# BogdanDIA/gr-dvbt

Measured on AMD Instinct MI355X. Metric: RX Msamples/s (baseband in -> TS out), higher is better.
Workload: dtype u8 (Viterbi/RS) + f32 (front end)

## Files before the change

gr_dvbt_amd/csrc/k_viterbi3.hpp:

```cpp
#pragma once
#include <hip/hip_runtime.h>
#include <stdint.h>
#include <limits.h>
#include <string.h>
#include "dvbt_tables.hpp"
#include "k_backend.hpp"

namespace dvbt {

inline VitParams make_vit_params(const Dims &d, int bsize, int chunk_bytes)
{
  VitParams v; memset(&v, 0, sizeof v);
  v.m = d.m; v.k = d.k; v.n = d.n; v.plen = d.plen; v.ntb = d.ntb; v.bsize = bsize;
  v.d_nsymbols = bsize * d.n / d.m; v.d_nbits = 2 * d.k * bsize;
  v.chunk_bytes = chunk_bytes > 0 ? chunk_bytes : 768; v.payload = d.payload; v.warm = 72;
  memcpy(v.punct, d.punct, 16); memcpy(v.prefix, d.prefix, 16);
  v.punct_mask = 0; v.prefix_nib = 0;
  for (int i = 0; i < d.plen; i++) { v.punct_mask |= (unsigned)d.punct[i] << i; v.prefix_nib |= (unsigned long long)d.prefix[i] << (4 * i); }
  v.magic_plen = ~0ull / (unsigned)d.plen + 1; v.magic_m = ~0ull / (unsigned)d.m + 1;
  for (int i = 0; i < 64; i++) v.punct_rep |= (unsigned long long)d.punct[i % d.plen] << i;
  v.magic16_plen = (65536u + (unsigned)d.plen - 1) / (unsigned)d.plen;
  return v;
}

#define DPP_XOR1 0xB1
#define DPP_XOR2 0x4E
#define DPP_HALF_MIRROR 0x141
#define DPP_ROR8 0x128
#define DPP_MIRROR 0x140

__device__ __forceinline__ int rotl6(int c, int p) { return ((c << p) | (c >> (6 - p))) & 63; }

#ifndef V3_WGW_N
#define V3_WGW_N 4
#endif
constexpr int V3_WGW = V3_WGW_N;
#ifndef V3_EXP
#define V3_EXP 0
#endif
constexpr int V3_WARM = 72;
constexpr int V3_WARM_MAX = 1152;
static_assert(V3_WARM == 72, "make_vit_params (above) presets VitParams.warm to the default");
constexpr int V3_BLK = 24;
constexpr int V3_RINGW = 64;
constexpr int V3_WAVES_PER_CU = 4 * 2;
constexpr int V3_CBW = 17;

typedef short v3pk __attribute__((ext_vector_type(2)));
__device__ __forceinline__ v3pk pk(int x) { return __builtin_bit_cast(v3pk, x); }
__device__ __forceinline__ int ipk(v3pk x) { return __builtin_bit_cast(int, x); }
__device__ __forceinline__ int pk_add(int a, int b) { return ipk(pk(a) + pk(b)); }
__device__ __forceinline__ int pk_sub(int a, int b) { return ipk(pk(a) - pk(b)); }
__device__ __forceinline__ int pk_max(int a, int b) { return ipk(__builtin_elementwise_max(pk(a), pk(b))); }
__device__ __forceinline__ int pk_min(int a, int b) { return ipk(__builtin_elementwise_min(pk(a), pk(b))); }
template <int CTRL> __device__ __forceinline__ int dppb(int v) { return __builtin_amdgcn_update_dpp(0, v, CTRL, 0xf, 0xf, true); }
__device__ __forceinline__ int vconst(int c) { int x; asm("v_mov_b32 %0, %1" : "=v"(x) : "s"(c)); return x; }
__device__ __forceinline__ int pk_max_swap(int a, int b) { int r; asm("v_pk_max_i16 %0, %1, %2 op_sel:[0,1] op_sel_hi:[1,0]" : "=v"(r) : "v"(a), "v"(b)); return r; }

struct V3Lane {
  unsigned sel[6][2];
  int bias8[6][2];
  int kc[3][2];
  int org[2];
  int arm_mid[3][2];
  int arm_b2[3][2];
  int arm_org[3][2];
};

__device__ __forceinline__ int v3_phys(int a) { const int a2 = (a >> 2) & 1; return (a & 8) | (a2 << 2) | ((a & 3) ^ (a2 ? 3 : 0)); }
__device__ __forceinline__ int v3_log(int p) { const int q = p & 7, a2 = (q >> 2) & 1; return (p & 8) | (a2 << 2) | ((q ^ (a2 ? 7 : 0)) & 3); }
__device__ __forceinline__ int v3_cell_of_z(int z) { return ((z & 2) << 4) | ((z & 1) << 4) | v3_log(z >> 2); }
__device__ __forceinline__ int v3_z_of_cell(int c) { return v3_phys(c & 15) * 4 + ((c >> 5) & 1) * 2 + ((c >> 4) & 1); }

__device__ __forceinline__ int v3_upper(int P, int r, int h, int a) { const int c = (r << 5) | (h << 4) | a; return (c >> (5 - P)) & 1; }
__device__ inline void v3_init_lane(int pl, V3Lane &L)
{
  const int a = v3_log(pl);
  for (int r = 0; r < 2; r++) {
    for (int P = 0; P < 6; P++) {
      unsigned idx[2];
      for (int h = 0; h < 2; h++) {
        const int c = (r << 5) | (h << 4) | a, i = rotl6(c, P) & 31;
        const int c0 = ((i >> 2) ^ (i >> 1) ^ i) & 1;
        const int c1 = ((i >> 4) ^ (i >> 2) ^ (i >> 1)) & 1;
        idx[h] = (unsigned)(c0 | (c1 << 1));
      }
      L.sel[P][r] = 0x0c | (idx[0] << 8) | (0x0cu << 16) | (idx[1] << 24);
      L.bias8[P][r] = (v3_upper(P, r, 0, a) << 8) | (v3_upper(P, r, 1, a) << 24);
    }
    L.org[r] = (pl * 4 + 2 * r) | ((pl * 4 + 2 * r + 1) << 16);
    for (int e = 0; e < 3; e++) {
      const int P0 = 2 * e;
      const int s0 = rotl6((r << 5) | a, P0), s1 = rotl6((r << 5) | 16 | a, P0);
      L.kc[e][r] = ((63 - s0) | ((63 - s1) << 16)) | (L.bias8[P0][r] ^ 0x01000100);
      const int b2 = ((s0 >> 4) << 6) | (((s1 >> 4) << 6) << 16);
      L.arm_mid[e][r] = (L.bias8[(P0 + 3) % 6][r] >> 2) | (L.bias8[(P0 + 4) % 6][r] >> 1) | L.bias8[(P0 + 5) % 6][r];
      L.arm_org[e][r] = L.org[r] | (L.bias8[P0][r] >> 2) | (L.bias8[P0 + 1][r] >> 1) | L.bias8[(P0 + 2) % 6][r];
      L.arm_b2[e][r] = b2 | L.bias8[P0][r];
    }
  }
  for (int r = 0; r < 2; r++) {
    for (int P = 0; P < 6; P++) asm("" : "+v"(L.bias8[P][r]));
    for (int e = 0; e < 3; e++) { asm("" : "+v"(L.kc[e][r])); asm("" : "+v"(L.arm_mid[e][r])); asm("" : "+v"(L.arm_b2[e][r])); asm("" : "+v"(L.arm_org[e][r])); }
  }
}

template <int P, int ST> __device__ __forceinline__ void v3_step(int (&v)[2], unsigned W, const V3Lane &L, int (&raw)[2])
{
  int X[2], Y[2], mx[2];
  const int D0 = (int)__builtin_amdgcn_perm(0u, W, L.sel[P][0]);
  X[0] = pk_add(v[0], D0); Y[0] = pk_sub(v[0], D0);
  if (P == 0 || P == 4) { X[1] = pk_add(v[1], D0); Y[1] = pk_sub(v[1], D0); }
  else if (P == 2 || P == 3) { X[1] = pk_sub(v[1], D0); Y[1] = pk_add(v[1], D0); }
  else {
    const int D1 = (int)__builtin_amdgcn_perm(0u, W, L.sel[P][1]);
    X[1] = pk_add(v[1], D1); Y[1] = pk_sub(v[1], D1);
  }
  if (P == 0) { mx[0] = pk_max(X[0], Y[1]); mx[1] = pk_max(X[1], Y[0]); }
  else if (P == 1) { mx[0] = pk_max_swap(X[0], Y[0]); mx[1] = pk_max_swap(X[1], Y[1]); }
  else {
#pragma unroll
    for (int r = 0; r < 2; r++)
      mx[r] = pk_max(X[r], P == 2 ? dppb<DPP_ROR8>(Y[r]) : P == 3 ? dppb<DPP_HALF_MIRROR>(Y[r]) : P == 4 ? dppb<DPP_XOR2>(Y[r]) : dppb<DPP_XOR1>(Y[r]));
  }
  constexpr int PN = (P + 1) % 6;
#pragma unroll
  for (int r = 0; r < 2; r++) {
    if (ST == 0) v[r] = mx[r];
    else if (ST == 3) v[r] = (mx[r] & (int)0xfe3ffe3f) | L.arm_mid[((PN + 3) % 6) / 2][r];
    else if (ST == 1) v[r] = (mx[r] & (int)0xfe3ffe3f) | L.arm_b2[PN / 2][r];
    else if (ST == 4) v[r] = (mx[r] & (int)0xfefffeff) | L.bias8[PN][r];
    else { raw[r] = mx[r]; v[r] = (mx[r] & (int)0xfe00fe00) | L.arm_org[PN / 2][r]; }
  }
}

#if V3_EXP & 64
#define V3_YIELD() asm volatile("s_nop 3" ::: "memory")
#else
#define V3_YIELD()
#endif

__device__ __forceinline__ int lo16(int x) { return (x << 16) >> 16; }
__device__ __forceinline__ int hi16(int x) { return x >> 16; }
template <int CTRL> __device__ __forceinline__ int max_dpp(int v) { return max(v, dppb<CTRL>(v)); }
template <int CTRL> __device__ __forceinline__ int min_dpp(int v) { return min(v, dppb<CTRL>(v)); }

template <int PE, bool RENORM> __device__ __forceinline__ int v3_window_end(int (&v)[2], const V3Lane &L)
{
  const int kp = pk_max((v[0] & (int)0xfe00fe00) | L.kc[PE / 2][0], (v[1] & (int)0xfe00fe00) | L.kc[PE / 2][1]);
  int k = max(lo16(kp), hi16(kp));
  k = max_dpp<DPP_XOR1>(k); k = max_dpp<DPP_XOR2>(k); k = max_dpp<DPP_HALF_MIRROR>(k); k = max_dpp<DPP_MIRROR>(k);
  if (RENORM) {
    const unsigned sub = (unsigned)((k & ~0x1ff) - (48 << 8));
    const int mn = (int)__builtin_amdgcn_perm(sub, sub, 0x01000100u);
    v[0] = pk_sub(v[0], mn); v[1] = pk_sub(v[1], mn);
  }
  return k;
}

template <int NW> constexpr int V3_ROW = NW * 4 * 64;
template <int NW> constexpr int V3_RMASK = (V3_RINGW * V3_ROW<NW> - 1) & ~63;
struct V3Trace {
  int z[2];
  int wsh[2];
  int oph[2];
  bool ok[2];
  int oend[2];
  int ob[2];
};
__device__ __forceinline__ void v3_hop_read(const V3Trace &T, const unsigned char *tab, unsigned (&t)[2])
{
#pragma unroll
  for (int q = 0; q < 2; q++) t[q] = tab[T.z[q]];
}
template <int NW> __device__ __forceinline__ void v3_hop_merge(V3Trace &T, const unsigned (&t)[2])
{
#pragma unroll
  for (int q = 0; q < 2; q++) {
    T.wsh[q] -= V3_ROW<NW>;
    asm("v_bfi_b32 %0, %1, %2, %3" : "=v"(T.z[q]) : "s"(V3_RMASK<NW>), "v"(T.wsh[q]), "v"(t[q]));
  }
}
template <int NW> __device__ __forceinline__ void v3_hop(V3Trace &T, const unsigned char *tab) { unsigned t[2]; v3_hop_read(T, tab, t); v3_hop_merge<NW>(T, t); }
__device__ __forceinline__ void v3_trace_out(const V3Trace &T, const unsigned char *tab, uint8_t *outb)
{
#pragma unroll
  for (int q = 0; q < 2; q++) {
    const unsigned t = tab[T.z[q]];
    const int sstart = rotl6(v3_cell_of_z((int)(t & 63u)), T.oph[q]);
    if (T.ok[q]) outb[T.ob[q]] = (unsigned char)((sstart << 2) | (t >> 6));
  }
}

__device__ __forceinline__ void v3_load_words(const unsigned *wp_, unsigned (&W)[8])
{
  const uint4 *wp = reinterpret_cast<const uint4 *>(wp_);
  const uint4 t0 = wp[0], t1 = wp[1];
  W[0] = t0.x; W[1] = t0.y; W[2] = t0.z; W[3] = t0.w; W[4] = t1.x; W[5] = t1.y; W[6] = t1.z; W[7] = t1.w;
}
template <int V6, bool HOPS, int HOP0, int NTB, int NW, bool PREF> __device__ __forceinline__ void v3_fwd_window(int (&v)[2], const V3Lane &L, const unsigned *wrow, unsigned char *tab, unsigned char *tabw,
                                                                                           unsigned char *bests, int j0, int dd, int pl, V3Trace &T, unsigned (&W)[8], unsigned (&Wn)[8])
{
  constexpr bool HOPA = HOPS && HOP0 + 2 * V6 < NTB - 1, HOPB = HOPS && HOP0 + 2 * V6 + 1 < NTB - 1;
  unsigned th[2];
  if (HOPA) v3_hop_read(T, tab, th);
  const int jr = (j0 + V6) & (V3_RINGW - 1);
#if V3_EXP & 256
  for (int i = 0; i < 8; i++) { W[i] = (unsigned)(j0 * 0x01010101 + i * 0x00020406 + pl); asm volatile("" : "+v"(W[i])); }
#else
  if (PREF) v3_load_words(wrow + (V6 + 1) * 8, Wn);
#endif
  constexpr int P0 = (8 * V6) % 6;
  int raw[2];
#if V3_EXP & 32
  if (V6 & 1) __builtin_amdgcn_s_setprio(1); else __builtin_amdgcn_s_setprio(0);
#endif
#if V3_EXP & 128
  __builtin_amdgcn_s_sleep(1);
#endif
  v3_step<(P0 + 0) % 6, 0>(v, W[0], L, raw); V3_YIELD(); v3_step<(P0 + 1) % 6, 0>(v, W[1], L, raw); V3_YIELD(); v3_step<(P0 + 2) % 6, 3>(v, W[2], L, raw); V3_YIELD();
  if (HOPA) { v3_hop_merge<NW>(T, th); if (HOPB) v3_hop_read(T, tab, th); }
  v3_step<(P0 + 3) % 6, 0>(v, W[3], L, raw); V3_YIELD(); v3_step<(P0 + 4) % 6, 0>(v, W[4], L, raw); V3_YIELD(); v3_step<(P0 + 5) % 6, 1>(v, W[5], L, raw); V3_YIELD();
  v3_step<(P0 + 6) % 6, 4>(v, W[6], L, raw); V3_YIELD(); v3_step<(P0 + 7) % 6, 2>(v, W[7], L, raw);
  if (HOPB) v3_hop_merge<NW>(T, th);
  if (!(V3_EXP & 4)) *reinterpret_cast<unsigned *>(tabw + jr * V3_ROW<NW>) = __builtin_amdgcn_perm((unsigned)raw[1], (unsigned)raw[0], 0x06040200u);
  if (V3_EXP & 2) { if (raw[0] == 0x12345) bests[jr] = 1; return; }
  const int s = v3_window_end<(P0 + 2) % 6, (V6 & 1) == 1>(v, L);
  bests[dd * V3_RINGW + jr] = (unsigned char)s;
}
template <bool HOPS, int HOP0, int NTB, int NW, bool MORE> __device__ __forceinline__ void v3_fwd_six(int (&v)[2], const V3Lane &L, const unsigned *wrow, unsigned char *tab, unsigned char *tabw,
                                                                                  unsigned char *bests, int j0, int dd, int pl, V3Trace &T, unsigned (&Wa)[8], unsigned (&Wb)[8])
{
  v3_fwd_window<0, HOPS, HOP0, NTB, NW, true>(v, L, wrow, tab, tabw, bests, j0, dd, pl, T, Wa, Wb); v3_fwd_window<1, HOPS, HOP0, NTB, NW, true>(v, L, wrow, tab, tabw, bests, j0, dd, pl, T, Wb, Wa);
  v3_fwd_window<2, HOPS, HOP0, NTB, NW, true>(v, L, wrow, tab, tabw, bests, j0, dd, pl, T, Wa, Wb); v3_fwd_window<3, HOPS, HOP0, NTB, NW, true>(v, L, wrow, tab, tabw, bests, j0, dd, pl, T, Wb, Wa);
  v3_fwd_window<4, HOPS, HOP0, NTB, NW, true>(v, L, wrow, tab, tabw, bests, j0, dd, pl, T, Wa, Wb); v3_fwd_window<5, HOPS, HOP0, NTB, NW, MORE>(v, L, wrow, tab, tabw, bests, j0, dd, pl, T, Wb, Wa);
}

#if V3_EXP & 16
__device__ unsigned long long *v3_dbg;
#endif

constexpr int V3_SLOT = 32;
constexpr int V3_CTL_CHUNKS = 0;
constexpr int V3_CTL_MISMATCH = 1;
constexpr int V3_CTL_CONFLICT = 2;
constexpr int V3_CTL_UNPROVEN = 3;
constexpr int V3_CTL_SEQ = 4;
constexpr int V3_CTL_ACC = 8;
constexpr int V3_CTL_HDR = 16;
struct V3Aux {
  int *snap;
  int *ctl;
  long long cap;
  long long grid0;
  const int *carry_in;
  int *carry_out; int carry_rel;
  int debug;
};
__device__ __forceinline__ int *v3_own(const V3Aux &ax, long long c) { return ax.snap + (3 * c) * V3_SLOT; }
__device__ __forceinline__ int *v3_pred(const V3Aux &ax, long long c) { return ax.snap + (3 * c + 1) * V3_SLOT; }
__device__ __forceinline__ int *v3_fix(const V3Aux &ax, long long c) { return ax.snap + (3 * c + 2) * V3_SLOT; }
inline size_t v3_snap_words(long long cap) { return (size_t)(cap + 2) * 3 * V3_SLOT; }
inline size_t v3_ctl_words(long long cap) { return (size_t)V3_CTL_HDR + 2 * (size_t)(cap + 2); }

struct V3Lds { unsigned char *tab; unsigned *wbuf; unsigned char *bests; const unsigned *lut; int wv; };
__device__ __forceinline__ void v3_init_lut(unsigned *lut, int lane)
{
  if (lane < 16) {
    const int k0 = (lane >> 2) & 1, k1 = (lane >> 3) & 1, t1 = (lane >> 1) & 1, t0 = lane & 1;
    const int u0 = k0 ? 1 - 2 * t1 : 0, u1 = k1 ? 1 - 2 * (k0 ? t0 : t1) : 0;
    const unsigned d0 = (unsigned)(2 * (u0 + u1)) & 0xff, d1 = (unsigned)(2 * (-u0 + u1)) & 0xff;
    const unsigned d2 = (unsigned)(2 * (u0 - u1)) & 0xff, d3 = (unsigned)(2 * (-u0 - u1)) & 0xff;
    lut[lane] = d0 | (d1 << 8) | (d2 << 16) | (d3 << 24);
  }
}

template <int NTB, int WARM, int MODE, int NW>
__device__ __forceinline__ void v3_decode(const uint8_t *__restrict__ in, uint8_t *__restrict__ out, long long total_steps, long long total_out, const VitParams &vp,
                                          long long in_base, long long out_lo, long long b0, bool dec_active, const V3Lds &S, const V3Lane &L, int (&v)[2], int (&endv)[2],
                                          int *own, int *predn, const int *inject, int *carry, int carry_rel)
{
  unsigned char *const tab = S.tab; unsigned *const wbuf = S.wbuf; unsigned char *const bests = S.bests; const unsigned *const lut = S.lut;
  unsigned *const cbits = wbuf;
  constexpr int V3_CBS = V3_BLK * 8;
  static_assert(V3_CBW <= V3_CBS, "bit stream does not fit the step-word row");
  const int lane = threadIdx.x & 63, dd = lane >> 4, pl = lane & 15;
  const int rowl = S.wv * 256 + dd * 64;
  unsigned char *const tabw = tab + rowl + pl * 4;
  const int B = vp.chunk_bytes, m = vp.m;
  constexpr int ntb = NTB;
  const long long b1 = (b0 + B < total_out) ? b0 + B : total_out;
  const int warm = MODE == 2 ? 0 : WARM > 0 ? WARM : vp.warm;
  const long long w0 = b0 + 2 - warm;
  const int J = ((warm + B + ntb - 1 + V3_BLK - 1) / V3_BLK) * V3_BLK;
  const long long n_in_bytes = (total_steps * 2 / vp.plen * vp.n + vp.m - 1) / vp.m;
  const int nload = ((384 + 2 * m - 2) / m + 3 + 15) / 16;

  uint8_t *const outb = out + (b0 - out_lo);
  const int ob_end = !dec_active ? INT_MIN : (int)(b1 - b0 > INT_MIN / 2 ? b1 - b0 : INT_MIN / 2);
  const int ob_lo = MODE != 1 || out_lo <= b0 ? 0 : (int)(out_lo - b0 < INT_MAX / 2 ? out_lo - b0 : INT_MAX / 2);
  const long long tb0 = 8 * (w0 - 1) - 2;
  constexpr int BLKBITS = 2 * 8 * V3_BLK;
  const int inc_q = BLKBITS / vp.plen, inc_ph = BLKBITS - inc_q * vp.plen;
  const unsigned magic16_m = (65536u + (unsigned)m - 1) / (unsigned)m;

  int u_first, u_last;
  {
    const long long r = total_steps - 8 * V3_BLK - tb0;
    int first = tb0 >= 0 ? 0 : (int)((-tb0 + 7) >> 3 < J ? (-tb0 + 7) >> 3 : J), last = !dec_active || r < 0 ? -1 : (int)(r >> 3 < J ? r >> 3 : J);
    u_first = max(max(__builtin_amdgcn_readlane(first, 0), __builtin_amdgcn_readlane(first, 16)), max(__builtin_amdgcn_readlane(first, 32), __builtin_amdgcn_readlane(first, 48)));
    u_last = min(min(__builtin_amdgcn_readlane(last, 0), __builtin_amdgcn_readlane(last, 16)), min(__builtin_amdgcn_readlane(last, 32), __builtin_amdgcn_readlane(last, 48)));
  }
  int ph0 = 0, bo0 = 0, off = 0; long long byte0 = 0; uint4 q = make_uint4(0, 0, 0, 0);
  auto stage_load = [&](int jb) {
    const long long tb = tb0 + (long long)jb * 8;
    if (jb > 0 && jb - V3_BLK >= u_first) {
      const int pf0 = (int)((vp.prefix_nib >> (4 * ph0)) & 15ull);
      ph0 += inc_ph;
      const int wrap = ph0 >= vp.plen ? 1 : 0;
      ph0 -= wrap ? vp.plen : 0;
      const int r = bo0 + (inc_q + wrap) * vp.n + (int)((vp.prefix_nib >> (4 * ph0)) & 15ull) - pf0;
      const int dby = (int)(((unsigned)r * magic16_m) >> 16);
      bo0 = r - dby * m; byte0 += dby;
    } else {
      const unsigned long long pbit = 2ull * (unsigned long long)(tb > 0 ? tb : 0);
      const unsigned long long pq = __umul64hi(pbit, vp.magic_plen);
      ph0 = (int)(pbit - pq * (unsigned)vp.plen);
      const unsigned long long rb = pq * (unsigned)vp.n + ((vp.prefix_nib >> (4 * ph0)) & 15ull);
      const unsigned long long by = __umul64hi(rb, vp.magic_m);
      byte0 = (long long)by; bo0 = (int)(rb - by * (unsigned)m);
    }
    off = (int)(((unsigned long long)(uintptr_t)in + (unsigned long long)(byte0 - in_base)) & 3ull);
    const long long src = byte0 - off + pl * 16;
    q = make_uint4(0, 0, 0, 0);
    if (dec_active && pl < nload) {
      if (src >= in_base && src + 16 <= n_in_bytes) q = *reinterpret_cast<const uint4 *>(in + (src - in_base));
      else {
        unsigned w[4] = {0, 0, 0, 0};
        for (int i = 0; i < 16; i++) {
          const long long bb = src + i;
          const unsigned bv = (bb >= in_base && bb < n_in_bytes) ? in[bb - in_base] : 0;
          w[i >> 2] |= bv << (8 * (i & 3));
        }
        q = make_uint4(w[0], w[1], w[2], w[3]);
      }
    }
  };
  auto stage_words = [&](int jb) {
    {
      const unsigned mk = (1u << m) - 1;
      auto grp = [&](unsigned d) { return ((d & mk) << (3 * m)) | (((d >> 8) & mk) << (2 * m)) | (((d >> 16) & mk) << m) | ((d >> 24) & mk); };
      const unsigned g0 = grp(q.x), g1 = grp(q.y), g2 = grp(q.z), g3 = grp(q.w);
      unsigned *cb = cbits + dd * V3_CBS;
      if (pl < nload) {
        if (m == 2) cb[pl] = (g0 << 24) | (g1 << 16) | (g2 << 8) | g3;
        else if (m == 4) { cb[2 * pl] = (g0 << 16) | g1; cb[2 * pl + 1] = (g2 << 16) | g3; }
        else { cb[3 * pl] = (g0 << 8) | (g1 >> 16); cb[3 * pl + 1] = (g1 << 16) | (g2 >> 8); cb[3 * pl + 2] = (g2 << 24) | g3; }
      }
    }
    __builtin_amdgcn_fence(__ATOMIC_SEQ_CST, "wavefront");
    constexpr int SPL = V3_BLK * 8 / 16;
    const long long tb = tb0 + (long long)jb * 8;
    const int ub0 = pl * SPL;
    int lo = 0, hi = SPL;
    int x = ph0 + 2 * ub0;
    if (jb < u_first || jb > u_last) {
      const long long tbr = tb > 0 ? tb : 0;
      const long long t = tb + ub0;
      if (t < 0) lo = (-t < SPL) ? (int)(-t) : SPL;
      const long long rem = total_steps - t;
      hi = !dec_active ? 0 : rem <= 0 ? 0 : rem < SPL ? (int)rem : SPL;
      if (hi < lo) hi = lo;
      x = ph0 + 2 * (int)((t + lo) - tbr);
      if (x < 0) x = 0;
    }
    const int dq = (int)(((unsigned)x * vp.magic16_plen) >> 16);
    const int ph = x - dq * vp.plen;
    const int pos = off * m + bo0 + dq * vp.n + (int)((vp.prefix_nib >> (4 * ph)) & 15ull) - (int)((vp.prefix_nib >> (4 * ph0)) & 15ull);
    const unsigned kmask = ((unsigned)(vp.punct_rep >> ph) << (2 * lo)) & (((1u << (2 * hi)) - 1u) & ~((1u << (2 * lo)) - 1u));
    const unsigned *cb = cbits + dd * V3_CBS;
    const unsigned cw0 = cb[pos >> 5], cw1 = cb[(pos >> 5) + 1];
    unsigned win = (unsigned)(((((unsigned long long)cw0) << 32) | cw1) >> (32 - (pos & 31)));
#pragma unroll
    for (int i = 0; i < SPL; i++) {
      const unsigned k2 = (kmask >> (2 * i)) & 3u;
      const unsigned idx = (k2 << 2) | (win >> 30);
      win <<= __popc(k2);
      wbuf[dd * (V3_BLK * 8) + ub0 + i] = lut[idx];
    }
    __builtin_amdgcn_fence(__ATOMIC_SEQ_CST, "wavefront");
  };
  V3Trace T;
  int tph[2];
#pragma unroll
  for (int c = 0; c < 2; c++) { T.oend[c] = c * 16 + pl < V3_BLK ? ob_end : INT_MIN; tph[c] = 2 * ((c * 16 + pl + 1) % 3); T.oph[c] = 2 * ((c * 16 + pl + 3 * ntb - (ntb - 1)) % 3); }
  static_assert(V3_BLK % 3 == 0, "phases per lane");
  auto trace_init = [&](int jp) {
#pragma unroll
    for (int c = 0; c < 2; c++) {
      const int jj = jp + c * 16 + pl;
      T.ob[c] = jj - (warm + ntb - 1);
      T.ok[c] = T.ob[c] >= ob_lo && T.ob[c] < T.oend[c];
      const int sb = 63 - (bests[dd * V3_RINGW + (jj & (V3_RINGW - 1))] & 63);
      T.wsh[c] = jj * V3_ROW<NW> + rowl;
      T.z[c] = v3_z_of_cell(((sb | (sb << 6)) >> tph[c]) & 63) | (T.wsh[c] & V3_RMASK<NW>);
    }
  };

  stage_load(0);
  for (int jb = 0; jb < J; jb += V3_BLK) {
    if (MODE == 1 && dec_active) {
      if (jb == warm) { if (inject) { v[0] = inject[0]; v[1] = inject[1]; } own[0] = v[0]; own[1] = v[1]; }
      if (jb == warm + B) { predn[0] = v[0]; predn[1] = v[1]; }
      if (carry && jb == warm + carry_rel) { carry[0] = v[0]; carry[1] = v[1]; }
    }
    if (MODE == 2) {
      if (jb == 0 && dec_active) { own[0] = v[0]; own[1] = v[1]; }
      if (jb == B) { endv[0] = v[0]; endv[1] = v[1]; }
      if (carry && dec_active && jb == carry_rel) { carry[0] = v[0]; carry[1] = v[1]; }
    }
    if (!(V3_EXP & 8) || jb == 0) stage_words(jb);
    if (jb + V3_BLK < J && !(V3_EXP & 8)) stage_load(jb + V3_BLK);
    const bool tr = jb > 0 && !(V3_EXP & 1);
    if (tr) trace_init(jb - V3_BLK);
    const unsigned *wrow = wbuf + dd * (V3_BLK * 8);
    unsigned Wa[8], Wb[8];
    v3_load_words(wrow, Wa);
    if (tr) {
      v3_fwd_six<true, 0, NTB, NW, true>(v, L, wrow, tab, tabw, bests, jb, dd, pl, T, Wa, Wb);
      v3_fwd_six<true, 12, NTB, NW, true>(v, L, wrow + 48, tab, tabw, bests, jb + 6, dd, pl, T, Wa, Wb);
      v3_trace_out(T, tab, outb);
    } else {
      v3_fwd_six<false, 0, NTB, NW, true>(v, L, wrow, tab, tabw, bests, jb, dd, pl, T, Wa, Wb);
      v3_fwd_six<false, 0, NTB, NW, true>(v, L, wrow + 48, tab, tabw, bests, jb + 6, dd, pl, T, Wa, Wb);
    }
    static_assert(V3_BLK == 24, "the second half of the block is written out: two groups of six windows, straight-line like the first half");
    v3_fwd_six<false, 0, NTB, NW, true>(v, L, wrow + 96, tab, tabw, bests, jb + 12, dd, pl, T, Wa, Wb);
    v3_fwd_six<false, 0, NTB, NW, false>(v, L, wrow + 144, tab, tabw, bests, jb + 18, dd, pl, T, Wa, Wb);
  }
  __builtin_amdgcn_fence(__ATOMIC_SEQ_CST, "wavefront");
  trace_init(J - V3_BLK);
  for (int h = 0; h < ntb - 1; h++) v3_hop<NW>(T, tab);
  v3_trace_out(T, tab, outb);
}

template <int NW> struct V3Shared {
  alignas(16) unsigned char tab[V3_RINGW * V3_ROW<NW>];
  alignas(16) unsigned wbuf[NW][4 * V3_BLK * 8];
  unsigned char bests[NW][4 * V3_RINGW];
  unsigned lut[16];
};
static_assert(sizeof(V3Shared<4>) <= 81920 && V3_RMASK<4> == 0xffc0 && V3_RMASK<1> == 0x3fc0, "two four-wave workgroups per CU beside the symbol kernel's 76 KB");
#define V3_LDS_DECL(NW) __shared__ V3Shared<NW> sh_;
#define V3_LDS(NW, wv) V3Lds{sh_.tab, sh_.wbuf[wv], sh_.bests[wv], sh_.lut, wv}

template <int NTB, int WARM = V3_WARM, int MODE = 0> __global__ __launch_bounds__(64 * V3_WGW) void viterbi3_kernel(const uint8_t *__restrict__ in, uint8_t *__restrict__ out, const RxState *st,
                                                      long long steps_fixed, VitParams vp, V3Aux ax, long long in_base, long long out_lo)
{
  V3_LDS_DECL(V3_WGW)
  const int wv = V3_WGW > 1 ? (int)(threadIdx.x >> 6) : 0;
  const V3Lds S = V3_LDS(V3_WGW, wv);
  const int lane = threadIdx.x & 63, dd = lane >> 4, pl = lane & 15;
  const long long total_steps = st ? st->n_vit_steps : steps_fixed;
  const long long total_out = total_steps / 8 - vp.ntb;
  const int B = vp.chunk_bytes;
  if (MODE == 1 && blockIdx.x == 0 && threadIdx.x == 0) {
    ax.ctl[V3_CTL_MISMATCH] = 0; ax.ctl[V3_CTL_CONFLICT] = 0; ax.ctl[V3_CTL_UNPROVEN] = -1; ax.ctl[V3_CTL_SEQ] = 0;
  }
  const long long grid0 = MODE == 1 ? ax.grid0 : out_lo;
  const long long chunk0 = ((long long)blockIdx.x * V3_WGW + wv) * 4;
  if (grid0 + chunk0 * B >= total_out) return;
  const long long c = chunk0 + dd, b0 = grid0 + c * B;
  const bool dec_active = b0 < total_out;
  v3_init_lut(sh_.lut, lane);
#if V3_EXP & 16
  const unsigned long long dbg_t0 = wall_clock64();
#endif
  V3Lane L; v3_init_lane(pl, L);
  int v[2] = {L.arm_org[0][0], L.arm_org[0][1]}, endv[2];
  int *own = nullptr, *predn = nullptr, *carry = nullptr; const int *inject = nullptr;
  if (MODE == 1) {
    own = v3_own(ax, c) + 2 * pl; predn = v3_pred(ax, c + 1) + 2 * pl;
    if (c == 0 && ax.carry_in) inject = ax.carry_in + 2 * pl;
    if (ax.carry_out && b0 + B >= total_out) carry = ax.carry_out + 2 * pl;
  }
  v3_decode<NTB, WARM, MODE, V3_WGW>(in, out, total_steps, total_out, vp, in_base, out_lo, b0, dec_active, S, L, v, endv, own, predn, inject, carry, ax.carry_rel);
#if V3_EXP & 16
  if (lane == 0) {
    unsigned id, xcc;
    asm volatile("s_getreg_b32 %0, hwreg(HW_REG_HW_ID)" : "=s"(id));
    asm volatile("s_getreg_b32 %0, hwreg(HW_REG_XCC_ID)" : "=s"(xcc));
    unsigned long long *d = v3_dbg + 3 * ((long long)blockIdx.x * V3_WGW + wv);
    d[0] = (id & 0xffffu) | ((xcc & 0xfu) << 16); d[1] = dbg_t0; d[2] = wall_clock64();
  }
#endif
}

__device__ __forceinline__ long long v3_nchunks(long long total_out, long long grid0, int B) { return total_out > grid0 ? (total_out - grid0 + B - 1) / B : 0; }
__device__ __forceinline__ bool v3_slots_equal(const int *a_, const int *b_)
{
  const int4 *a = reinterpret_cast<const int4 *>(a_), *b = reinterpret_cast<const int4 *>(b_);
  bool same = true;
#pragma unroll
  for (int i = 0; i < 8; i++) { const int4 x = a[i], y = b[i]; same = same && x.x == y.x && x.y == y.y && x.z == y.z && x.w == y.w; }
  return same;
}

__global__ __launch_bounds__(256) void viterbi_check_kernel(V3Aux ax, const RxState *st, long long steps_fixed, VitParams vp, int pass)
{
  const long long total_steps = st ? st->n_vit_steps : steps_fixed;
  const long long nch = v3_nchunks(total_steps / 8 - vp.ntb, ax.grid0, vp.chunk_bytes);
  if (blockIdx.x == 0 && threadIdx.x == 0) { ax.ctl[V3_CTL_CHUNKS] = (int)(nch < INT_MAX ? nch : INT_MAX); if (pass == 1) ax.ctl[V3_CTL_UNPROVEN] = 0; }
  const long long c = (long long)blockIdx.x * 256 + threadIdx.x + 1;
  if (c >= nch || c > ax.cap) return;
  const bool same = v3_slots_equal(v3_own(ax, c), v3_pred(ax, c));
  if (pass == 0) {
    ax.ctl[V3_CTL_HDR + (ax.cap + 2) + c] = 0;
    if (!same) ax.ctl[V3_CTL_HDR + atomicAdd(ax.ctl + V3_CTL_MISMATCH, 1)] = (int)c;
  }
}
__global__ __launch_bounds__(256) void viterbi_count_kernel(V3Aux ax, const RxState *st, long long steps_fixed, VitParams vp)
{
  const long long total_steps = st ? st->n_vit_steps : steps_fixed;
  const long long nch = v3_nchunks(total_steps / 8 - vp.ntb, ax.grid0, vp.chunk_bytes);
  const long long c = (long long)blockIdx.x * 256 + threadIdx.x + 1;
  if (c >= nch || c > ax.cap) return;
  if (!v3_slots_equal(v3_own(ax, c), v3_pred(ax, c))) atomicAdd(ax.ctl + V3_CTL_UNPROVEN, 1);
}

__device__ __forceinline__ bool v3_row_equal(const int (&a)[2], const int (&b)[2], int dd)
{
  const unsigned long long ne = __ballot(a[0] != b[0] || a[1] != b[1]);
  return ((ne >> (16 * dd)) & 0xffffull) == 0;
}

template <int NTB, int NW> __device__ __forceinline__ void v3_repair_rows(const uint8_t *__restrict__ in, uint8_t *__restrict__ out, long long total_steps, const VitParams &vp, const V3Aux &ax,
                                                                  long long in_base, long long out_lo, const V3Lds &S, const V3Lane &L, long long rows, long long row0, int n)
{
  const int lane = threadIdx.x & 63, dd = lane >> 4, pl = lane & 15;
  const long long total_out = total_steps / 8 - vp.ntb;
  const int B = vp.chunk_bytes;
  const long long nch = v3_nchunks(total_out, ax.grid0, B);
  for (long long i0 = row0; i0 < n; i0 += rows) {
    const bool act = i0 + dd < n;
    const long long c = act ? ax.ctl[V3_CTL_HDR + i0 + dd] : 1;
    const long long b0 = ax.grid0 + c * B;
    int v[2], endv[2] = {0, 0};
    { const int *p = v3_pred(ax, c) + 2 * pl; v[0] = p[0]; v[1] = p[1]; }
    int *carry = (act && ax.carry_out && b0 + B >= total_out) ? ax.carry_out + 2 * pl : nullptr;
    v3_decode<NTB, 0, 2, NW>(in, out, total_steps, total_out, vp, in_base, out_lo, b0, act && b0 < total_out, S, L, v, endv, v3_own(ax, c) + 2 * pl, nullptr, nullptr, carry, ax.carry_rel);
    int pn[2] = {endv[0], endv[1]};
    if (act && c + 1 < nch) { const int *p = v3_pred(ax, c + 1) + 2 * pl; pn[0] = p[0]; pn[1] = p[1]; }
    if (!v3_row_equal(endv, pn, dd) || ((ax.debug & 1) && act && c + 1 < nch)) {
      int *f = v3_fix(ax, c + 1) + 2 * pl; f[0] = endv[0]; f[1] = endv[1];
      if (pl == 0) { ax.ctl[V3_CTL_HDR + (ax.cap + 2) + c + 1] = 1; atomicAdd(ax.ctl + V3_CTL_CONFLICT, 1); }
    }
    __builtin_amdgcn_fence(__ATOMIC_SEQ_CST, "wavefront");
  }
}
template <int NTB> __global__ __launch_bounds__(64 * V3_WGW) void viterbi_repair_kernel(const uint8_t *__restrict__ in, uint8_t *__restrict__ out, const RxState *st,
                                                      long long steps_fixed, VitParams vp, V3Aux ax, long long in_base, long long out_lo)
{
  V3_LDS_DECL(V3_WGW)
  const int n = ax.ctl[V3_CTL_MISMATCH];
  const int wv = V3_WGW > 1 ? (int)(threadIdx.x >> 6) : 0;
  const long long rows = (long long)gridDim.x * V3_WGW * 4, row0 = ((long long)blockIdx.x * V3_WGW + wv) * 4;
  if (row0 >= n) return;
  const V3Lds S = V3_LDS(V3_WGW, wv);
  v3_init_lut(sh_.lut, threadIdx.x & 63);
  V3Lane L; v3_init_lane(threadIdx.x & 15, L);
  v3_repair_rows<NTB, V3_WGW>(in, out, st ? st->n_vit_steps : steps_fixed, vp, ax, in_base, out_lo, S, L, rows, row0, n);
}

template <int NTB, int NW> __device__ __forceinline__ void v3_seq_walk(const uint8_t *__restrict__ in, uint8_t *__restrict__ out, long long total_steps, const VitParams &vp, const V3Aux &ax,
                                                               long long in_base, long long out_lo, const V3Lds &S, const V3Lane &L, int force)
{
  const int lane = threadIdx.x & 63, dd = lane >> 4, pl = lane & 15;
  if (lane == 0) { ax.ctl[V3_CTL_ACC] += ax.ctl[V3_CTL_CHUNKS]; ax.ctl[V3_CTL_ACC + 1] += ax.ctl[V3_CTL_MISMATCH]; }
  if (!force && ax.ctl[V3_CTL_CONFLICT] == 0) return;
  const long long total_out = total_steps / 8 - vp.ntb;
  const int B = vp.chunk_bytes;
  long long nch = v3_nchunks(total_out, ax.grid0, B);
  if (nch > ax.cap) nch = ax.cap;
  const int *cflag = ax.ctl + V3_CTL_HDR + (ax.cap + 2);
  int done = 0;
  long long pos = 0;
  for (;;) {
    long long cn = -1;
    for (long long c0 = pos + 1; c0 < nch && cn < 0; c0 += 64) {
      const long long c = c0 + lane;
      bool hit = false;
      if (c < nch) hit = cflag[c] != 0 || (force && !v3_slots_equal(v3_own(ax, c), v3_pred(ax, c)));
      const unsigned long long b = __ballot(hit);
      if (b) cn = c0 + __builtin_ctzll(b);
    }
    if (cn < 0) break;
    long long c = cn;
    int v[2];
    { const int *p = (cflag[c] ? v3_fix(ax, c) : v3_pred(ax, c)) + 2 * pl; v[0] = p[0]; v[1] = p[1]; }
    for (;;) {
      const long long b0 = ax.grid0 + c * B;
      const bool act = dd == 0;
      int st0[2] = {v[0], v[1]}, endv[2] = {0, 0};
      if (act) { int *p = v3_pred(ax, c) + 2 * pl; p[0] = v[0]; p[1] = v[1]; }
      int *carry = (act && ax.carry_out && b0 + B >= total_out) ? ax.carry_out + 2 * pl : nullptr;
      v3_decode<NTB, 0, 2, NW>(in, out, total_steps, total_out, vp, in_base, out_lo, b0, act, S, L, st0, endv, v3_own(ax, c) + 2 * pl, nullptr, nullptr, carry, ax.carry_rel);
      __builtin_amdgcn_fence(__ATOMIC_SEQ_CST, "wavefront");
      done++;
      if (c + 1 >= nch) { pos = nch; break; }
      int on[2]; { const int *p = v3_own(ax, c + 1) + 2 * pl; on[0] = p[0]; on[1] = p[1]; }
      const bool eq = (__ballot(on[0] != endv[0] || on[1] != endv[1]) & 0xffffull) == 0;
      if (act) { int *p = v3_pred(ax, c + 1) + 2 * pl; p[0] = endv[0]; p[1] = endv[1]; }
      if (eq) { pos = c + 1; break; }
      c++; v[0] = endv[0]; v[1] = endv[1];
    }
  }
  if (lane == 0) { ax.ctl[V3_CTL_SEQ] = done; ax.ctl[V3_CTL_ACC + 2] += done; }
}
template <int NTB> __global__ __launch_bounds__(64) void viterbi_repair_seq_kernel(const uint8_t *__restrict__ in, uint8_t *__restrict__ out, const RxState *st,
                                                      long long steps_fixed, VitParams vp, V3Aux ax, long long in_base, long long out_lo, int force)
{
  V3_LDS_DECL(1)
  const V3Lds S = V3_LDS(1, 0);
  v3_init_lut(sh_.lut, threadIdx.x & 63);
  V3Lane L; v3_init_lane(threadIdx.x & 15, L);
  v3_seq_walk<NTB, 1>(in, out, st ? st->n_vit_steps : steps_fixed, vp, ax, in_base, out_lo, S, L, force);
}

constexpr long long V3_FIX_SMALL = 1024;
template <int NTB> __global__ __launch_bounds__(64 * V3_WGW) void viterbi_fix_kernel(const uint8_t *__restrict__ in, uint8_t *__restrict__ out, const RxState *st,
                                                      long long steps_fixed, VitParams vp, V3Aux ax, long long in_base, long long out_lo, int force)
{
  V3_LDS_DECL(V3_WGW)
  const int wv = V3_WGW > 1 ? (int)(threadIdx.x >> 6) : 0;
  const long long total_steps = st ? st->n_vit_steps : steps_fixed;
  const long long nch = v3_nchunks(total_steps / 8 - vp.ntb, ax.grid0, vp.chunk_bytes);
  if (threadIdx.x == 0) ax.ctl[V3_CTL_CHUNKS] = (int)(nch < INT_MAX ? nch : INT_MAX);
  for (long long c = 1 + threadIdx.x; c < nch && c <= ax.cap; c += 64 * V3_WGW) {
    ax.ctl[V3_CTL_HDR + (ax.cap + 2) + c] = 0;
    if (!v3_slots_equal(v3_own(ax, c), v3_pred(ax, c))) ax.ctl[V3_CTL_HDR + atomicAdd(ax.ctl + V3_CTL_MISMATCH, 1)] = (int)c;
  }
  __threadfence(); __syncthreads();
  const int n = *(volatile int *)(ax.ctl + V3_CTL_MISMATCH);
  const V3Lds S = V3_LDS(V3_WGW, wv);
  v3_init_lut(sh_.lut, threadIdx.x & 63);
  V3Lane L; v3_init_lane(threadIdx.x & 15, L);
  if (!force && n > 0) v3_repair_rows<NTB, V3_WGW>(in, out, total_steps, vp, ax, in_base, out_lo, S, L, 4 * V3_WGW, 4 * wv, n);
  __threadfence(); __syncthreads();
  if (wv == 0) v3_seq_walk<NTB, V3_WGW>(in, out, total_steps, vp, ax, in_base, out_lo, S, L, force);
}

}
```

Measured before the change: 36760.

## Fold traceback output into hop slots and vectorize step-word staging stores

The final traceback read and byte store now go into the forward-window schedule at the hop slot where each chain finishes, instead of running as a separate tail after the two six-window groups. The output mask becomes a wave ballot and is applied with an exec-masked inline-asm store. Several smaller changes come with it: the puncture prefix is computed from a popcount instead of a nibble-table lookup, the per-lane LUT words are written to LDS as 16-byte stores, the bests read is hoisted ahead of staging, and the cell/z remapping is rewritten as XOR arithmetic. The inline asm that changes exec and the rewritten bit mappings carry correctness risk.

```diff
diff --git a/gr_dvbt_amd/csrc/k_viterbi3.hpp b/gr_dvbt_amd/csrc/k_viterbi3.hpp
--- a/gr_dvbt_amd/csrc/k_viterbi3.hpp
+++ b/gr_dvbt_amd/csrc/k_viterbi3.hpp
@@ -163,8 +163,8 @@
 struct V3Trace {
   int z[2];
   int wsh[2];
-  int oph[2];
-  bool ok[2];
+  int osh[2];
+  unsigned long long ok[2];
   int oend[2];
   int ob[2];
 };
@@ -182,15 +182,24 @@
   }
 }
 template <int NW> __device__ __forceinline__ void v3_hop(V3Trace &T, const unsigned char *tab) { unsigned t[2]; v3_hop_read(T, tab, t); v3_hop_merge<NW>(T, t); }
-__device__ __forceinline__ void v3_trace_out(const V3Trace &T, const unsigned char *tab, uint8_t *outb)
+__device__ __forceinline__ void v3_trace_read(const V3Trace &T, const unsigned char *tab, unsigned (&t)[2])
+{
+#pragma unroll
+  for (int q = 0; q < 2; q++) t[q] = tab[T.z[q]];
+}
+template <bool MASKED> __device__ __forceinline__ void v3_trace_store(const V3Trace &T, const unsigned (&t)[2], uint8_t *outb)
 {
 #pragma unroll
   for (int q = 0; q < 2; q++) {
-    const unsigned t = tab[T.z[q]];
-    const int sstart = rotl6(v3_cell_of_z((int)(t & 63u)), T.oph[q]);
-    if (T.ok[q]) outb[T.ob[q]] = (unsigned char)((sstart << 2) | (t >> 6));
-  }
-}
+    const unsigned zz = (t[q] ^ (((t[q] >> 4) & 1u) * 12u)) & 63u;
+    unsigned by = (((zz | (zz << 6)) >> T.osh[q]) & 0xfcu) | (t[q] >> 6);
+    if (MASKED) {
+      unsigned long long sv;
+      asm volatile("s_and_saveexec_b64 %0, %1\n\tglobal_store_byte %2, %3, off\n\ts_mov_b64 exec, %0" : "=&s"(sv) : "s"(T.ok[q]), "v"(outb + T.ob[q]), "v"(by) : "memory", "scc");
+    } else if ((T.ok[q] >> (threadIdx.x & 63)) & 1) outb[T.ob[q]] = (unsigned char)by;
+  }
+}
+__device__ __forceinline__ void v3_trace_out(const V3Trace &T, const unsigned char *tab, uint8_t *outb) { unsigned t[2]; v3_trace_read(T, tab, t); v3_trace_store<false>(T, t, outb); }
 
 __device__ __forceinline__ void v3_load_words(const unsigned *wp_, unsigned (&W)[8])
 {
@@ -199,11 +208,13 @@
   W[0] = t0.x; W[1] = t0.y; W[2] = t0.z; W[3] = t0.w; W[4] = t1.x; W[5] = t1.y; W[6] = t1.z; W[7] = t1.w;
 }
 template <int V6, bool HOPS, int HOP0, int NTB, int NW, bool PREF> __device__ __forceinline__ void v3_fwd_window(int (&v)[2], const V3Lane &L, const unsigned *wrow, unsigned char *tab, unsigned char *tabw,
-                                                                                           unsigned char *bests, int j0, int dd, int pl, V3Trace &T, unsigned (&W)[8], unsigned (&Wn)[8])
+                                                                                           unsigned char *bests, int j0, int dd, int pl, V3Trace &T, unsigned (&W)[8], unsigned (&Wn)[8], uint8_t *outb)
 {
   constexpr bool HOPA = HOPS && HOP0 + 2 * V6 < NTB - 1, HOPB = HOPS && HOP0 + 2 * V6 + 1 < NTB - 1;
-  unsigned th[2];
+  constexpr bool FINA = HOPS && HOP0 + 2 * V6 == NTB - 1, FINB = HOPS && HOP0 + 2 * V6 + 1 == NTB - 1;
+  unsigned th[2], tout[2];
   if (HOPA) v3_hop_read(T, tab, th);
+  if (FINA) v3_trace_read(T, tab, tout);
   const int jr = (j0 + V6) & (V3_RINGW - 1);
 #if V3_EXP & 256
   for (int i = 0; i < 8; i++) { W[i] = (unsigned)(j0 * 0x01010101 + i * 0x00020406 + pl); asm volatile("" : "+v"(W[i])); }
@@ -220,20 +231,23 @@
 #endif
   v3_step<(P0 + 0) % 6, 0>(v, W[0], L, raw); V3_YIELD(); v3_step<(P0 + 1) % 6, 0>(v, W[1], L, raw); V3_YIELD(); v3_step<(P0 + 2) % 6, 3>(v, W[2], L, raw); V3_YIELD();
   if (HOPA) { v3_hop_merge<NW>(T, th); if (HOPB) v3_hop_read(T, tab, th); }
+  if (FINB) v3_trace_read(T, tab, tout);
+  if (FINA) v3_trace_store<true>(T, tout, outb);
   v3_step<(P0 + 3) % 6, 0>(v, W[3], L, raw); V3_YIELD(); v3_step<(P0 + 4) % 6, 0>(v, W[4], L, raw); V3_YIELD(); v3_step<(P0 + 5) % 6, 1>(v, W[5], L, raw); V3_YIELD();
   v3_step<(P0 + 6) % 6, 4>(v, W[6], L, raw); V3_YIELD(); v3_step<(P0 + 7) % 6, 2>(v, W[7], L, raw);
   if (HOPB) v3_hop_merge<NW>(T, th);
+  if (FINB) v3_trace_store<true>(T, tout, outb);
   if (!(V3_EXP & 4)) *reinterpret_cast<unsigned *>(tabw + jr * V3_ROW<NW>) = __builtin_amdgcn_perm((unsigned)raw[1], (unsigned)raw[0], 0x06040200u);
   if (V3_EXP & 2) { if (raw[0] == 0x12345) bests[jr] = 1; return; }
   const int s = v3_window_end<(P0 + 2) % 6, (V6 & 1) == 1>(v, L);
   bests[dd * V3_RINGW + jr] = (unsigned char)s;
 }
 template <bool HOPS, int HOP0, int NTB, int NW, bool MORE> __device__ __forceinline__ void v3_fwd_six(int (&v)[2], const V3Lane &L, const unsigned *wrow, unsigned char *tab, unsigned char *tabw,
-                                                                                  unsigned char *bests, int j0, int dd, int pl, V3Trace &T, unsigned (&Wa)[8], unsigned (&Wb)[8])
-{
-  v3_fwd_window<0, HOPS, HOP0, NTB, NW, true>(v, L, wrow, tab, tabw, bests, j0, dd, pl, T, Wa, Wb); v3_fwd_window<1, HOPS, HOP0, NTB, NW, true>(v, L, wrow, tab, tabw, bests, j0, dd, pl, T, Wb, Wa);
-  v3_fwd_window<2, HOPS, HOP0, NTB, NW, true>(v, L, wrow, tab, tabw, bests, j0, dd, pl, T, Wa, Wb); v3_fwd_window<3, HOPS, HOP0, NTB, NW, true>(v, L, wrow, tab, tabw, bests, j0, dd, pl, T, Wb, Wa);
-  v3_fwd_window<4, HOPS, HOP0, NTB, NW, true>(v, L, wrow, tab, tabw, bests, j0, dd, pl, T, Wa, Wb); v3_fwd_window<5, HOPS, HOP0, NTB, NW, MORE>(v, L, wrow, tab, tabw, bests, j0, dd, pl, T, Wb, Wa);
+                                                                                  unsigned char *bests, int j0, int dd, int pl, V3Trace &T, unsigned (&Wa)[8], unsigned (&Wb)[8], uint8_t *outb)
+{
+  v3_fwd_window<0, HOPS, HOP0, NTB, NW, true>(v, L, wrow, tab, tabw, bests, j0, dd, pl, T, Wa, Wb, outb); v3_fwd_window<1, HOPS, HOP0, NTB, NW, true>(v, L, wrow, tab, tabw, bests, j0, dd, pl, T, Wb, Wa, outb);
+  v3_fwd_window<2, HOPS, HOP0, NTB, NW, true>(v, L, wrow, tab, tabw, bests, j0, dd, pl, T, Wa, Wb, outb); v3_fwd_window<3, HOPS, HOP0, NTB, NW, true>(v, L, wrow, tab, tabw, bests, j0, dd, pl, T, Wb, Wa, outb);
+  v3_fwd_window<4, HOPS, HOP0, NTB, NW, true>(v, L, wrow, tab, tabw, bests, j0, dd, pl, T, Wa, Wb, outb); v3_fwd_window<5, HOPS, HOP0, NTB, NW, MORE>(v, L, wrow, tab, tabw, bests, j0, dd, pl, T, Wb, Wa, outb);
 }
 
 #if V3_EXP & 16
@@ -311,22 +325,24 @@
     u_first = max(max(__builtin_amdgcn_readlane(first, 0), __builtin_amdgcn_readlane(first, 16)), max(__builtin_amdgcn_readlane(first, 32), __builtin_amdgcn_readlane(first, 48)));
     u_last = min(min(__builtin_amdgcn_readlane(last, 0), __builtin_amdgcn_readlane(last, 16)), min(__builtin_amdgcn_readlane(last, 32), __builtin_amdgcn_readlane(last, 48)));
   }
-  int ph0 = 0, bo0 = 0, off = 0; long long byte0 = 0; uint4 q = make_uint4(0, 0, 0, 0);
+  auto pfx = [&](int ph) { return (int)__popc(vp.punct_mask & ((1u << ph) - 1u)); };
+  int ph0 = 0, pf0 = 0, bo0 = 0, off = 0; long long byte0 = 0; uint4 q = make_uint4(0, 0, 0, 0);
   auto stage_load = [&](int jb) {
     const long long tb = tb0 + (long long)jb * 8;
     if (jb > 0 && jb - V3_BLK >= u_first) {
-      const int pf0 = (int)((vp.prefix_nib >> (4 * ph0)) & 15ull);
+      const int pf_old = pf0;
       ph0 += inc_ph;
       const int wrap = ph0 >= vp.plen ? 1 : 0;
       ph0 -= wrap ? vp.plen : 0;
-      const int r = bo0 + (inc_q + wrap) * vp.n + (int)((vp.prefix_nib >> (4 * ph0)) & 15ull) - pf0;
+      pf0 = pfx(ph0);
+      const int r = bo0 + (inc_q + wrap) * vp.n + pf0 - pf_old;
       const int dby = (int)(((unsigned)r * magic16_m) >> 16);
       bo0 = r - dby * m; byte0 += dby;
     } else {
       const unsigned long long pbit = 2ull * (unsigned long long)(tb > 0 ? tb : 0);
       const unsigned long long pq = __umul64hi(pbit, vp.magic_plen);
-      ph0 = (int)(pbit - pq * (unsigned)vp.plen);
-      const unsigned long long rb = pq * (unsigned)vp.n + ((vp.prefix_nib >> (4 * ph0)) & 15ull);
+      ph0 = (int)(pbit - pq * (unsigned)vp.plen); pf0 = pfx(ph0);
+      const unsigned long long rb = pq * (unsigned)vp.n + (unsigned)pf0;
       const unsigned long long by = __umul64hi(rb, vp.magic_m);
       byte0 = (long long)by; bo0 = (int)(rb - by * (unsigned)m);
     }
@@ -376,36 +392,49 @@
     }
     const int dq = (int)(((unsigned)x * vp.magic16_plen) >> 16);
     const int ph = x - dq * vp.plen;
-    const int pos = off * m + bo0 + dq * vp.n + (int)((vp.prefix_nib >> (4 * ph)) & 15ull) - (int)((vp.prefix_nib >> (4 * ph0)) & 15ull);
+    const int pos = off * m + bo0 + dq * vp.n + pfx(ph) - pf0;
     const unsigned kmask = ((unsigned)(vp.punct_rep >> ph) << (2 * lo)) & (((1u << (2 * hi)) - 1u) & ~((1u << (2 * lo)) - 1u));
     const unsigned *cb = cbits + dd * V3_CBS;
     const unsigned cw0 = cb[pos >> 5], cw1 = cb[(pos >> 5) + 1];
     unsigned win = (unsigned)(((((unsigned long long)cw0) << 32) | cw1) >> (32 - (pos & 31)));
+    unsigned idx[SPL], sw[SPL];
 #pragma unroll
     for (int i = 0; i < SPL; i++) {
       const unsigned k2 = (kmask >> (2 * i)) & 3u;
-      const unsigned idx = (k2 << 2) | (win >> 30);
+      idx[i] = (k2 << 2) | (win >> 30);
       win <<= __popc(k2);
-      wbuf[dd * (V3_BLK * 8) + ub0 + i] = lut[idx];
-    }
+    }
+#pragma unroll
+    for (int i = 0; i < SPL; i++) sw[i] = lut[idx[i]];
+    static_assert(SPL % 4 == 0, "a lane's step words are whole 16-byte groups (its offset dd * 768 + pl * 48 bytes is 16-byte aligned)");
+    uint4 *const wdst = reinterpret_cast<uint4 *>(wbuf + dd * (V3_BLK * 8) + ub0);
+#pragma unroll
+    for (int i = 0; i < SPL / 4; i++) wdst[i] = make_uint4(sw[4 * i], sw[4 * i + 1], sw[4 * i + 2], sw[4 * i + 3]);
     __builtin_amdgcn_fence(__ATOMIC_SEQ_CST, "wavefront");
   };
   V3Trace T;
-  int tph[2];
-#pragma unroll
-  for (int c = 0; c < 2; c++) { T.oend[c] = c * 16 + pl < V3_BLK ? ob_end : INT_MIN; tph[c] = 2 * ((c * 16 + pl + 1) % 3); T.oph[c] = 2 * ((c * 16 + pl + 3 * ntb - (ntb - 1)) % 3); }
+  int tsh[2];
+#pragma unroll
+  for (int c = 0; c < 2; c++) {
+    T.oend[c] = c * 16 + pl < V3_BLK ? ob_end : INT_MIN; tsh[c] = (2 * ((c * 16 + pl + 1) % 3) + 4) % 6; T.osh[c] = (6 - 2 * ((c * 16 + pl + 3 * ntb - (ntb - 1)) % 3)) % 6;
+  }
   static_assert(V3_BLK % 3 == 0, "phases per lane");
-  auto trace_init = [&](int jp) {
+  auto bests_read = [&](int jp, unsigned (&bb)[2]) {
+#pragma unroll
+    for (int c = 0; c < 2; c++) bb[c] = bests[dd * V3_RINGW + ((jp + c * 16 + pl) & (V3_RINGW - 1))];
+  };
+  auto trace_init = [&](int jp, const unsigned (&bb)[2]) {
 #pragma unroll
     for (int c = 0; c < 2; c++) {
       const int jj = jp + c * 16 + pl;
       T.ob[c] = jj - (warm + ntb - 1);
-      T.ok[c] = T.ob[c] >= ob_lo && T.ob[c] < T.oend[c];
-      const int sb = 63 - (bests[dd * V3_RINGW + (jj & (V3_RINGW - 1))] & 63);
+      T.ok[c] = __builtin_amdgcn_ballot_w64(T.ob[c] >= ob_lo && T.ob[c] < T.oend[c]);
       T.wsh[c] = jj * V3_ROW<NW> + rowl;
-      T.z[c] = v3_z_of_cell(((sb | (sb << 6)) >> tph[c]) & 63) | (T.wsh[c] & V3_RMASK<NW>);
+      const unsigned R = (bb[c] | (bb[c] << 6)) >> tsh[c];
+      T.z[c] = (int)((R ^ 51u ^ (((R >> 4) & 1u) * 12u)) & 63u) | (T.wsh[c] & V3_RMASK<NW>);
     }
   };
+  unsigned bb[2];
 
   stage_load(0);
   for (int jb = 0; jb < J; jb += V3_BLK) {
@@ -419,27 +448,29 @@
       if (jb == B) { endv[0] = v[0]; endv[1] = v[1]; }
       if (carry && dec_active && jb == carry_rel) { carry[0] = v[0]; carry[1] = v[1]; }
     }
+    bests_read(jb - V3_BLK, bb);
     if (!(V3_EXP & 8) || jb == 0) stage_words(jb);
     if (jb + V3_BLK < J && !(V3_EXP & 8)) stage_load(jb + V3_BLK);
     const bool tr = jb > 0 && !(V3_EXP & 1);
-    if (tr) trace_init(jb - V3_BLK);
+    if (tr) trace_init(jb - V3_BLK, bb);
     const unsigned *wrow = wbuf + dd * (V3_BLK * 8);
     unsigned Wa[8], Wb[8];
     v3_load_words(wrow, Wa);
     if (tr) {
-      v3_fwd_six<true, 0, NTB, NW, true>(v, L, wrow, tab, tabw, bests, jb, dd, pl, T, Wa, Wb);
-      v3_fwd_six<true, 12, NTB, NW, true>(v, L, wrow + 48, tab, tabw, bests, jb + 6, dd, pl, T, Wa, Wb);
-      v3_trace_out(T, tab, outb);
+      v3_fwd_six<true, 0, NTB, NW, true>(v, L, wrow, tab, tabw, bests, jb, dd, pl, T, Wa, Wb, outb);
+      v3_fwd_six<true, 12, NTB, NW, true>(v, L, wrow + 48, tab, tabw, bests, jb + 6, dd, pl, T, Wa, Wb, outb);
     } else {
-      v3_fwd_six<false, 0, NTB, NW, true>(v, L, wrow, tab, tabw, bests, jb, dd, pl, T, Wa, Wb);
-      v3_fwd_six<false, 0, NTB, NW, true>(v, L, wrow + 48, tab, tabw, bests, jb + 6, dd, pl, T, Wa, Wb);
+      v3_fwd_six<false, 0, NTB, NW, true>(v, L, wrow, tab, tabw, bests, jb, dd, pl, T, Wa, Wb, outb);
+      v3_fwd_six<false, 0, NTB, NW, true>(v, L, wrow + 48, tab, tabw, bests, jb + 6, dd, pl, T, Wa, Wb, outb);
     }
     static_assert(V3_BLK == 24, "the second half of the block is written out: two groups of six windows, straight-line like the first half");
-    v3_fwd_six<false, 0, NTB, NW, true>(v, L, wrow + 96, tab, tabw, bests, jb + 12, dd, pl, T, Wa, Wb);
-    v3_fwd_six<false, 0, NTB, NW, false>(v, L, wrow + 144, tab, tabw, bests, jb + 18, dd, pl, T, Wa, Wb);
+    static_assert(NTB - 1 < 24, "the chains' last read takes a hop slot of the first twelve windows");
+    v3_fwd_six<false, 0, NTB, NW, true>(v, L, wrow + 96, tab, tabw, bests, jb + 12, dd, pl, T, Wa, Wb, outb);
+    v3_fwd_six<false, 0, NTB, NW, false>(v, L, wrow + 144, tab, tabw, bests, jb + 18, dd, pl, T, Wa, Wb, outb);
   }
   __builtin_amdgcn_fence(__ATOMIC_SEQ_CST, "wavefront");
-  trace_init(J - V3_BLK);
+  bests_read(J - V3_BLK, bb);
+  trace_init(J - V3_BLK, bb);
   for (int h = 0; h < ntb - 1; h++) v3_hop<NW>(T, tab);
   v3_trace_out(T, tab, outb);
 }
```

After: 37500, median of 6. +2.0%, better.
